# marbl/parsnp

Hardware: AMD Instinct MI355X
Metric: genomes/sec (MUM+LCB end-to-end) (higher is better)
Workload: dtype int32

## Files before the change

### parsnp_amd/csrc/engine/engine_core.h

```cpp
#pragma once
#include <algorithm>
#include <atomic>
#include <chrono>
#include <cstdint>
#include <cstdio>
#include <cstdlib>
#include <cstring>
#include <memory>
#include <mutex>
#include <new>
#include <string>
#include <thread>
#include <vector>

#include "kernels.h"
#include "store_kernels.h"
#include "dense_kernels.h"
#include "index_kernels.h"

namespace pm {

struct HostPool {
    void* (*alloc_fn)(size_t) = nullptr;
    void (*free_fn)(void*) = nullptr;
// ... 669 lines not shown
            ensure(d_okcnt, (size_t)ncand + 1); ensure(d_okpos, (size_t)ncand + 1);
            be.launch("ok_count", (int64_t)ncand + 1, OkCount{d_ok.p, ncand_p, d_okcnt.p, (int64_t)ncand});
            be.exclusive_scan(d_okcnt.p, d_okpos.p, (size_t)ncand + 1);
            const int64_t* nok_p = d_okpos.p + ncand;
            int64_t nok = 0;
            if (exact) be.d2h(&nok, nok_p, 8);
            const size_t nokz = exact ? (size_t)nok : (size_t)ncand, nqz2 = (size_t)nq, ngz = (size_t)ngen;
            ensure(d_creg, std::max<size_t>(nokz, 1)); ensure(d_ck, std::max<size_t>(nokz, 1)); ensure(d_clon, std::max<size_t>(nokz, 1));
            std::vector<int32_t> reg_h(nokz);
            out->release();
            out->kb = pool->take(4 * nokz); out->lonb = pool->take(4 * nokz);
            out->rows = want_rows; out->dirty_known = false; out->table_id = 0; out->store_base = -1;
            const int64_t ms_before = ms_count, rg_before = rg_count, lay_before = layout_rows, pkey_before = rg_pkey_init;
            bool anchor_call = false;
            if (!want_rows) {
                ensure(d_csp, std::max<size_t>(nokz * nqz2, 1)); ensure(d_cfwd, std::max<size_t>(nokz * nqz2, 1));
                be.launch("compact_sp", (int64_t)ncand * nq,
                          CompactSp{scand, d_ok.p, d_okpos.p, nq, d_ok_k.p, d_ok_lon.p, d_osp.p, d_ofwd.p, d_creg.p, d_ck.p, d_clon.p, d_csp.p, d_cfwd.p, ncand_p});
                be.mark("download");
                group_downloads();
                out->spb = pool->take(4 * nokz * nqz2); out->fwdb = pool->take(nokz * nqz2);
                be.d2h_async(out->spb.p, d_csp.p, 4 * nokz * nqz2);
                be.d2h_async(out->fwdb.p, d_cfwd.p, nokz * nqz2);
            } else {
                anchor_call = nreg == 1 && !gb && (exact ? nok >= dirty_min : anchor_guess);
                const bool keep_rows = resident && (anchor_call || from_store);
                const bool to_store = anchor_call || keep_rows;
                int32_t* p_start; uint8_t* p_strand; int32_t* p_lon; uint32_t* p_flags;
                if (to_store) {
                    if (anchor_call) { ms_count = 0; rg_count = 0; layout_rows = -1; rg_pkey_init = 0; }
                    const size_t base = (size_t)ms_count, upto = base + nokz;
                    ensure_keep(d_anchor_start, std::max<size_t>(upto * ngz, 1), base * ngz); ensure_keep(d_ms_strand, std::max<size_t>(upto * ngz, 1), base * ngz);
                    ensure_keep(d_anchor_lon, std::max<size_t>(upto, 1), base); ensure_keep(d_anchor_flags, std::max<size_t>(upto, 1), base);
                    ensure_keep(d_ms_shift, std::max<size_t>(upto, 1), base); ensure_keep(d_ms_len, std::max<size_t>(upto, 1), base); ensure_keep(d_ms_state, std::max<size_t>(upto, 1), base);
                    p_start = d_anchor_start.p + base * ngz; p_strand = d_ms_strand.p + base * ngz; p_lon = d_anchor_lon.p + base; p_flags = d_anchor_flags.p + base;
                    out->store_base = (int64_t)base;
                    ms_count = (int64_t)upto;
                } else {
                    ensure(d_csp, std::max<size_t>(nokz * ngz, 1)); ensure(d_cfwd, std::max<size_t>(nokz * ngz, 1)); ensure(d_cflags, std::max<size_t>(nokz, 1));
                    p_start = d_csp.p; p_strand = d_cfwd.p; p_lon = d_clon.p; p_flags = d_cflags.p;
                }
                const bool long_list = nreg == 1 && (exact ? nok >= dirty_min : anchor_guess);
                if (long_list) ensure(d_dirty, nokz);
                {
                    const ClearJob jobs[] = {{p_flags, 4 * nokz, 0}, {long_list ? d_dirty.p : nullptr, long_list ? 4 * nokz : 0, 0},
                                             {to_store ? d_ms_shift.p + (ms_count - (int64_t)nokz) : nullptr, to_store ? 4 * nokz : 0, 0},
                                             {to_store ? d_ms_state.p + (ms_count - (int64_t)nokz) : nullptr, to_store ? nokz : 0, 0}};
                    be.clear_many(jobs, 4);
                }
                be.launch("compact_candidates", (int64_t)ncand * ngen,
                          CompactCandidates{scand, d_ok.p, d_okpos.p, ngen, d_ok_k.p, d_ok_lon.p, d_osp.p, d_ofwd.p, d_starts.p, d_lens.p, d_glen,
                                            d_creg.p, d_ck.p, p_lon, p_start, p_strand, p_flags, ncand_p});
                if (long_list) {
                    const int64_t nblocks = ((int64_t)nokz + kDirtyBlock - 1) / kDirtyBlock, groups = (ngen + 63) / 64;
                    ensure(d_bmax, (size_t)nblocks * ngz); ensure(d_bmin, (size_t)nblocks * ngz);
                    be.launch_wave("dirty_extent", nblocks * groups, DirtyExtent{p_start, p_lon, p_flags, nok_p, ngen, d_bmax.p, d_bmin.p});
                    be.launch_wave("dirty_prefix", groups, DirtyPrefix{nblocks, ngen, d_bmax.p, d_bmin.p});
                    be.launch_wave("dirty_mark", nblocks * groups, DirtyMark{p_start, p_lon, nok_p, ngen, d_bmax.p, d_bmin.p, p_flags, d_dirty.p});
                    be.launch("dirty_merge", (int64_t)nokz, DirtyMerge{d_dirty.p, p_flags, nok_p});
                    out->dirty_known = true;
                }
                if (to_store) {
                    be.d2d(d_ms_len.p + (ms_count - (int64_t)nokz), p_lon, 4 * nokz);
                    if (anchor_call) out->table_id = ++table_counter;
                }
                be.mark("download");
                group_downloads();
                out->flagsb = pool->take(4 * nokz);
                be.d2h_async(out->flagsb.p, p_flags, 4 * nokz);
                if (!keep_rows) {
                    out->startb = pool->take(4 * nokz * ngz); out->strandb = pool->take(nokz * ngz);
                    be.d2h_async(out->startb.p, p_start, 4 * nokz * ngz);
                    be.d2h_async(out->strandb.p, p_strand, nokz * ngz);
                }
                be.d2h_async(out->lonb.p, p_lon, 4 * nokz);
            }
            if (!want_rows) be.d2h_async(out->lonb.p, d_clon.p, 4 * nokz);
            be.d2h_async(reg_h.data(), d_creg.p, 4 * nokz);
            be.d2h_async(out->kb.p, d_ck.p, 4 * nokz);
            int64_t counts_h[2] = {ncand_i, nok};
            if (!exact) { be.d2h_async(&counts_h[0], ncand_p, 8); be.d2h_async(&counts_h[1], nok_p, 8); }
            flush_downloads();
            be.mark(nullptr);
            be.sync();
            if (!exact) {
                ncand_i = counts_h[0]; nok = counts_h[1];
                const bool fits = (uint64_t)ncand_i <= ncand && anchor_call == (nreg == 1 && !gb && nok >= dirty_min);
                if (!fits) {
                    ms_count = ms_before; rg_count = rg_before; layout_rows = lay_before; rg_pkey_init = pkey_before;
                    tail_repeats++;
                    be.mark("candidates");
                    continue;
                }
                last_candidates = ncand_i;
                if (out->store_base >= 0) ms_count = out->store_base + nok;
            }
            hint.ncand = std::max<int64_t>(ncand_i, 1); hint.nok = nok;
            last_accepted = nok;
            if (anchor_call) { anchor_table_rows = nok; anchor_table_id = out->table_id; }
            for (int64_t w = 0; w < nok; w++) out->off[(size_t)reg_h[(size_t)w] + 1]++;
            for (int64_t r = 0; r < nreg; r++) out->off[(size_t)r + 1] += out->off[(size_t)r];
            out->total = out->off[(size_t)nreg];
            if (out->table_id && out->store_base == 0) anchor_flags_h.assign(out->flags(), out->flags() + nok);
            break;
        }
        collect_timing();
        return 0;
    }


    bool resident = false;
    int64_t ms_count = 0;
    int64_t rg_count = 0;
    std::vector<RegInfo> rg_info_h;
    std::vector<uint32_t> anchor_flags_h;
    static constexpr int kAgain = -6;

    void begin_store_call() { timing.clear(); last_events = last_rest = last_positions = last_candidates = last_accepted = last_grouped = last_grouped_wide = last_wide_regions = 0; last_handed_back = -1; last_index_bucketed = last_index_overflow = 0; last_index_lost = -1; last_alg[0] = last_alg[1] = last_alg[2] = 0; }
    Store store_view() { return Store{d_anchor_start.p, d_ms_strand.p, d_anchor_lon.p, d_anchor_flags.p, d_ms_shift.p, d_ms_len.p, d_ms_state.p, ngen}; }
    Layout layout_view(uint64_t* image, bool coherent = true) { return Layout{image, d_lay_off.p, d_lay_bits.p, coherent ? 1 : 0}; }
    size_t layout_geometry() {
        const size_t ngz = (size_t)ngen;
        if (lay_words == 0) {
            std::vector<int64_t> off(ngz + 1, 0), bits(ngz);
            for (size_t j = 0; j < ngz; j++) { bits[j] = glen_h[j] + 1; off[j + 1] = off[j] + (bits[j] + 63) / 64 + 1; }
            ensure(d_lay_off, ngz + 1); ensure(d_lay_bits, ngz);
            be.h2d(d_lay_off.p, off.data(), 8 * (ngz + 1)); be.h2d(d_lay_bits.p, bits.data(), 8 * ngz);
            lay_words = (size_t)off[ngz];
            lay_off_h = off;
        }
        return lay_words;
    }
    int need_resident(int64_t table_id) {
        if (!resident) { error = "the session is not in resident mode"; return -2; }
        if (table_id == 0 || table_id != anchor_table_id) { error = "the anchor table of this request is no longer resident"; return -2; }
        return 0;
    }
    int store_settle(int64_t table_id, RowInfo* out) {
        if (int rc = settle_launch(table_id)) return rc;
        return store_info(0, anchor_table_rows, out);
    }
    int settle_launch(int64_t table_id) {
        if (int rc = need_resident(table_id)) return rc;
        begin_store_call();
        const int64_t rows = anchor_table_rows;
        const size_t words = layout_geometry();
        ensure(d_image, words);
        be.mark("settle");
        ensure(d_foreign_count, 2);
        be.memset(d_foreign_count.p, 0, 16);
        ms_key_rows = 0; foreign_seen = 0;
        be.memset(d_image.p, 0, 8 * words);
        ensure(d_recwords, words);
        be.memset(d_recwords.p, 0, words);
        const Store S = store_view();
        const Layout L = layout_view(d_image.p);
        be.launch_wave("settle_clean", rows, SettleClean{S, P});
        std::vector<int32_t> fl;
        for (int64_t c = 0; c < rows; c++) { const uint32_t f = anchor_flags_h[(size_t)c]; if (!(f & (kRowBad | kRowOutside)) && (f & kRowDirty)) fl.push_back((int32_t)c); }
        const bool many_flagged = flagged_div > 1 && fl.size() * (size_t)flagged_div > (size_t)rows;
        bool ordered = true;
        for (int64_t c = 0; c < rows && ordered; c++) { const uint32_t f = anchor_flags_h[(size_t)c]; ordered = !((f & kRowEarly) && !(f & (kRowBad | kRowOutside | kRowDirty))); }
        if (ordered && !force_atomic_marks) be.launch_wave("store_mark_ordered", ((rows + kMarkRows - 1) / kMarkRows) * ((ngen + 63) / 64), StoreMarkOrdered{S, L, rows});
        else be.launch("store_mark", rows * ngen, StoreMark{S, L, 0, (uint8_t)(kStAccepted | kStFlagged), kStAccepted});
        be.launch("layout_sentinel", (int64_t)ngen, LayoutSentinel{d_lay_off.p, d_lay_bits.p, d_image.p});
        if (!fl.empty()) {
            const uint64_t* before_once = d_once.p; const uint64_t* before_twice = d_twice.p;
            ensure(d_once, words); ensure(d_twice, words); ensure(d_list, fl.size());
            if (d_once.p != before_once || d_twice.p != before_twice) { be.memset(d_once.p, 0, 8 * words); be.memset(d_twice.p, 0, 8 * words); }
            be.h2d(d_list.p, fl.data(), 4 * fl.size());
            be.launch("collide_mark", (int64_t)fl.size() * ngen, CollideMark{S, d_list.p, layout_view(d_once.p), d_twice.p});
            be.launch_wave("collide_test", (int64_t)fl.size(), CollideTest{S, d_list.p, layout_view(d_twice.p, false)});
            be.launch("collide_clear", (int64_t)fl.size() * ngen, CollideClear{S, d_list.p, layout_view(d_once.p), d_twice.p});
            ensure(d_t_rem, 2); ensure(d_t_done, fl.size());
            {
                const ClearJob jobs[] = {{d_t_rem.p, 16, 0}, {d_t_done.p, fl.size(), 0}};
                be.clear_many(jobs, 2);
            }
            be.launch("count_tangled", (int64_t)fl.size(), CountTangled{S, d_list.p, d_t_rem.p});
            if (many_flagged) {
                uint64_t tangled = 0;
                be.d2h(&tangled, d_t_rem.p, 8);
                if ((int64_t)tangled > tangled_max) {
                    be.mark(nullptr);
                    collect_timing_more();
                    error = "too many rows of the list overlap one another (rearranged genomes): the host route decides";
                    return kAgain;
                }
            }
            be.launch_wave("settle_flagged", (int64_t)fl.size(), SettleFlagged{S, layout_view(d_image.p, false), P, d_list.p});
            {
                const int32_t* before = d_owner.p;
                ensure(d_owner, words);
                if (d_owner.p != before) be.memset(d_owner.p, 0, 4 * words);
            }
            int rounds = tangle_rounds ? kTangleRounds : 0;
            if (rounds && tangle_ran > 0) {
                int last = 0;
                for (int r = 1; r < tangle_ran; r++) if (tangle_left[r] < tangle_left[r - 1]) last = r;
                rounds = std::min(kTangleRounds, last + 2);
            }
            ensure(d_t_left, kTangleRounds);
            for (int round = 0; round < rounds; round++) {
                be.launch_wave("tangle_owner", (int64_t)fl.size(), TangleOwner{S, d_list.p, d_lay_off.p, d_lay_bits.p, d_owner.p, d_t_done.p, d_t_rem.p});
                be.launch_wave("tangle_settle", (int64_t)fl.size(), TangleSettle{S, layout_view(d_image.p, false), P, d_list.p, d_owner.p, d_t_done.p, d_t_rem.p});
                be.launch_wave("tangle_clear", (int64_t)fl.size(), TangleClear{S, d_list.p, d_lay_off.p, d_lay_bits.p, d_owner.p, d_t_done.p, d_t_rem.p, d_t_left.p + round});
            }
            tangle_ran = 0;
            if (rounds) { be.d2h_async(tangle_left, d_t_left.p, 8 * (size_t)rounds); tangle_ran = rounds; }
            be.launch_wave("settle_tangled", 1, SettleTangled{S, L, P, d_list.p, (int64_t)fl.size(), d_t_done.p, d_t_rem.p});
        }
        layout_rows = rows;
        return 0;
    }
    int store_settle_seeds(int64_t table_id, int32_t q, RowInfo* out, std::vector<RegInfo>* infos, std::vector<int32_t>* ids) {
        infos->clear(); ids->clear();
// ... 500 lines not shown
            be.launch("dense_keys", n, DenseKeys{d_dstart.p, nflag, d_drank[k].p, (int64_t)1 << k, d_dkey.p, d_dval.p});
            be.sort_pairs(d_dkey.p, d_dkey2.p, d_dval.p, d_dval2.p, (size_t)n, 32 + bits_for(top_rank));
            be.launch("dense_heads", n + 1, DenseHeads{d_dkey2.p, n, d_dhead.p});
            be.exclusive_scan(d_dhead.p, d_dfirst.p, (size_t)n + 1);
            ensure(d_drank[k + 1], (size_t)n);
            be.launch("dense_rerank", n, DenseRerank{d_dval2.p, d_dhead.p, d_dfirst.p, d_drank[k + 1].p});
            L.lv[k + 1] = d_drank[k + 1].p;
            be.d2h(&groups, d_dfirst.p + n, 8);
            if (groups == n) break;
        }
        if (groups != n) { error = "suffix-array sort did not converge"; return -5; }
        dense_rounds = k + 1;
        L.top = k;
        be.launch("dense_lcp", n, DenseLcp{L, d_dval2.p, d_dstart.p, nflag, d_dlcp.p});
        be.launch("dense_rep", n, DenseRep{d_R.p, d_dlist.p, d_dval2.p, d_dstart.p, nflag, d_dlcp.p, d_rep.p});
        return 0;
    }
    bool dense_mode = false;
    std::vector<uint8_t> dense_h;
    void collect_timing_more() { for (const PhaseTime& t : be.collect()) timing.push_back(t); }

    int allgather_host(const void* send, int64_t bytes, void* recv) {
        if (!coll.device) return coll.allgather(coll.ctx, send, bytes, recv);
        ensure(d_hsend, (size_t)bytes); ensure(d_hrecv, (size_t)bytes * (size_t)coll.world);
        be.h2d(d_hsend.p, send, (size_t)bytes);
        if (be.allgather_dev(d_hsend.p, bytes, d_hrecv.p)) return 1;
        be.d2h(recv, d_hrecv.p, (size_t)bytes * (size_t)coll.world);
        return 0;
    }

    std::vector<uint64_t> ev_key_h, ev_val_h;
    std::vector<int32_t> rep_h;
    int ev_lbits = 0;
    int64_t work_budget = 1 << 22;
    int64_t dirty_min = 4096;
    int64_t flagged_div = 8;
    int64_t tangled_max = 1 << 17;
    bool fast_tail = true;
    int64_t tail_repeats = 0;
    bool tangle_rounds = true;
    bool group_small = true;
    bool group_wide = false;
    int64_t last_grouped = 0;
    int64_t last_grouped_wide = 0, last_handed_back = -1, last_wide_regions = 0;
    bool force_atomic_marks = false;
    int filter_factor = 8;
    int slot_factor = 2;
    bool bucket_sort = true;
    bool index_build = true;
    int64_t index_bucket_min = 1 << 24;
    bool index_verify = false;
    int64_t index_overflow_cap = 0;
    int64_t last_index_bucketed = 0, last_index_overflow = 0, last_index_lost = -1;
    bool master_seg = true;
    bool force_gate = false;
    int64_t chain_window = 4096;
    int64_t chain_passed[2] = {-1, -1};
    bool force_chain_tie = false;
    bool force_unsure = false;
    bool order_debug = false;
    int64_t outside_writes = 0;
    int64_t exact_cluster_tests = 0;
    int64_t deferred_regions = 0;
    bool clusters_out_of_order = false;
    int64_t hint_shrink = 1;
    bool phase_timing = true;
    bool tune(const std::string& key, int64_t value) {
        if (key == "flagged_div" && value >= 1) { flagged_div = value; return true; }
        if (key == "tangled_max" && value >= 0) { tangled_max = value; return true; }
        if (key == "tangle_rounds") { tangle_rounds = value != 0; return true; }
        if (key == "fast_tail") { fast_tail = value != 0; return true; }
        if (key == "atomic_marks") { force_atomic_marks = value != 0; return true; }
        if (key == "master_seg") { master_seg = value != 0; return true; }
        if (key == "bucket_sort") { bucket_sort = value != 0; return true; }
        if (key == "index_build") { index_build = value != 0; return true; }
        if (key == "index_bucket_min" && value >= 1) { index_bucket_min = value; return true; }
        if (key == "index_verify") { index_verify = value != 0; return true; }
        if (key == "index_overflow_cap" && value >= 0) { index_overflow_cap = value; return true; }
        if (key == "filter_factor") { filter_factor = value < 1 ? 1 : (int)value; return true; }
        if (key == "slot_factor") { slot_factor = value < 1 ? 1 : (int)value; return true; }
        if (key == "stage_gate") { force_gate = value != 0; return true; }
        if (key == "chain_window" && value >= 1 && value <= kChainWindowMax) { chain_window = value; return true; }
        if (key == "chain_tie") { force_chain_tie = value != 0; return true; }
        if (key == "cluster_unsure") { force_unsure = value != 0; return true; }
        if (key == "order_debug") { order_debug = value != 0; return true; }
        if (key == "timing") { phase_timing = value != 0; be.timing_on = phase_timing; return true; }
        if (key == "group_small") { group_small = value != 0; return true; }
        if (key == "group_wide") { group_wide = value != 0; return true; }
        if (key == "work_budget" && value > 0) { work_budget = value; return true; }
        if (key == "dense_all") { dense_all = value != 0; return true; }
        if (key == "dirty_min" && value >= 0) { dirty_min = value; return true; }
        if (key == "hint_shrink" && value >= 1) { hint_shrink = value; return true; }
        if (key == "copy_kernel") { return tune_copy_kernel(be, value != 0, 0); }
        return false;
    }

    void release() {
        if (chain_event) { be.event_wait(chain_event); be.event_release(chain_event); chain_event = nullptr; }
        for (BufBase* b : all_bufs) { if (b->raw) be.free(b->raw); b->raw = nullptr; b->cap = 0; }
        if (chain_host) be.pinned_free(chain_host);
        chain_host = nullptr; chain_host_cap = 0; chain_pending = false;
        if (blk) be.free(blk);
        if (d_goff) be.free(d_goff);
        if (d_glen) be.free(d_glen);
        blk = nullptr; d_goff = nullptr; d_glen = nullptr;
    }

    struct DeviceOutOfMemory { size_t bytes; };

private:
    B& be;
    struct BufBase { void* raw = nullptr; size_t cap = 0; };
    std::vector<BufBase*> all_bufs;
    template <class T> struct Buf : BufBase {
        T* p = nullptr;
    };
    template <class T> void ensure(Buf<T>& b, size_t n) {
        if (n <= b.cap && b.p) return;
        if (std::find(all_bufs.begin(), all_bufs.end(), (BufBase*)&b) == all_bufs.end()) all_bufs.push_back(&b);
        if (b.raw) be.free(b.raw);
        b.raw = nullptr; b.p = nullptr; b.cap = 0;
        const size_t want = n + n / 4 + 16;
        b.raw = be.alloc(want * sizeof(T));
        if (!b.raw) throw DeviceOutOfMemory{want * sizeof(T)};
        b.p = (T*)b.raw; b.cap = want;
    }
    template <class T> void ensure_keep(Buf<T>& b, size_t n, size_t keep) {
        if (n <= b.cap && b.p) return;
        if (std::find(all_bufs.begin(), all_bufs.end(), (BufBase*)&b) == all_bufs.end()) all_bufs.push_back(&b);
        const size_t want = n + n / 2 + 16;
        void* raw = be.alloc(want * sizeof(T));
        if (!raw) throw DeviceOutOfMemory{want * sizeof(T)};
        if (b.p && keep) { be.d2d(raw, b.p, keep * sizeof(T)); be.sync(); }
        if (b.raw) be.free(b.raw);
        b.raw = raw; b.p = (T*)raw; b.cap = want;
    }
    void collect_timing() { timing = be.collect(); }
    template <class T> static auto group_on(T& b, int) -> decltype(b.d2h_group(), void()) { b.d2h_group(); }
    template <class T> static void group_on(T&, long) {}
    template <class T> static auto flush_on(T& b, int) -> decltype(b.d2h_flush(), void()) { b.d2h_flush(); }
    template <class T> static void flush_on(T&, long) {}
    template <class T> static auto tune_copy_kernel(T& b, bool on, int) -> decltype(b.group_copies = on, true) { b.group_copies = on; return true; }
    template <class T> static bool tune_copy_kernel(T&, bool, long) { return true; }
    template <class T> static auto sort_keys_on(T& b, uint64_t* ki, uint64_t* ko, size_t n, int lo, int hi, int) -> decltype(b.sort_keys(ki, ko, n, lo, hi), true) { b.sort_keys(ki, ko, n, lo, hi); return true; }
    template <class T> static bool sort_keys_on(T&, uint64_t*, uint64_t*, size_t, int, int, long) { return false; }
    void group_downloads() { group_on(be, 0); }
    void flush_downloads() { flush_on(be, 0); }

    SeqBlock* blk = nullptr; int64_t* d_goff = nullptr; int64_t* d_glen = nullptr;
    int64_t total_words = 0;
    Packed P{};
    size_t ev_cap_hint = 0, cand_cap_hint = 0, rest_cap_hint[2] = {0, 0}, grp_cap_hint = 0;
    struct CallHint { int64_t units = 0, ncand = 0, nok = 0; };
    std::vector<CallHint> call_hints;
    int64_t call_ordinal = 0;
    Buf<uint8_t> d_gflag; Buf<int64_t> d_glo;
    Buf<int64_t> d_bkbase, d_bkbegin, d_ovf; Buf<uint64_t> d_ikey, d_ikey2, d_ikey3, d_ikey4;
    Buf<RegionInfo> d_R; Buf<int64_t> d_starts, d_lens, d_posbase;
    Buf<uint64_t> d_slots; Buf<uint32_t> d_filter, d_repeated; Buf<int32_t> d_next, d_rep, d_run, d_epm;
    Buf<int64_t> d_ucount, d_uoff; Buf<UnitRec> d_units;
    Buf<uint64_t> d_counter, d_evkey, d_evval, d_evkey2, d_evval2, d_evkey3, d_evval3; Buf<int64_t> d_sliceoff;
    Buf<int64_t> d_lo, d_cov; Buf<EventAtK> d_state; Buf<PairState> d_wsummary; Buf<int32_t> d_emax;
    Buf<uint64_t> d_cand; Buf<GenomeAtK> d_at; Buf<uint8_t> d_ok; Buf<int32_t> d_ok_k, d_ok_lon, d_osp; Buf<uint8_t> d_ofwd;
    Buf<uint64_t> d_wmask; Buf<int64_t> d_wcount, d_woff;
    Buf<int64_t> d_bcount, d_bbegin, d_pbase;
    Buf<int64_t> d_okcnt, d_okpos, d_cbase; Buf<int32_t> d_coarse; Buf<int32_t> d_creg, d_ck, d_clon, d_csp; Buf<uint8_t> d_cfwd;
    Buf<uint32_t> d_cflags, d_dirty; Buf<int32_t> d_bmax, d_bmin;
    Buf<GenomeAtK> d_xsend, d_xrecv; Buf<uint8_t> d_hsend, d_hrecv;
    Buf<RestItem> d_rest; Buf<uint64_t> d_qcount;
    Buf<uint8_t> d_dense; Buf<int32_t> d_dfi, d_dlist, d_dlcp; Buf<int64_t> d_dstart, d_dhead, d_dfirst;
    Buf<uint64_t> d_dkey, d_dkey2, d_dval, d_dval2; Buf<uint32_t> d_drank[kDenseMaxLevels];
    Buf<int32_t> d_anchor_start, d_anchor_lon; Buf<uint32_t> d_anchor_flags;
    int64_t table_counter = 0;
    Buf<uint64_t> d_image;
    Buf<uint8_t> d_ms_strand, d_ms_state, d_small8, d_o_strand; Buf<int32_t> d_ms_shift, d_ms_len, d_list, d_list2, d_j_min, d_j_max, d_o_start;
    Buf<int64_t> d_rg_start, d_rg_len, d_lay_off, d_lay_bits, d_v_row0, d_v_first, d_f_start, d_f_end, d_f_pack; Buf<RegInfo> d_rg_info; Buf<uint64_t> d_rg_count, d_once, d_twice;
    Buf<RowInfo> d_rowinfo; Buf<uint64_t> d_alg;
    Buf<int64_t> d_sd_cnt, d_sd_off; Buf<uint8_t> d_sd_keep;
    Buf<uint64_t> d_t_rem; Buf<uint8_t> d_t_done;
    Buf<int32_t> d_v_done, d_owner; Buf<uint8_t> d_v_defer, d_v_involved;
    Buf<uint64_t> d_t_left; uint64_t tangle_left[8] = {0, 0, 0, 0, 0, 0, 0, 0}; int tangle_ran = 0;
    Buf<int64_t> d_rg_pkey; Buf<OutsideWrite> d_outw; Buf<uint64_t> d_outw_count; int64_t rg_pkey_init = 0; uint64_t outside_writes_call = 0;
    Buf<ForeignRead> d_foreign; Buf<uint64_t> d_foreign_count, d_foreign_masks; Buf<int64_t> d_ms_key;
    size_t foreign_cap = 0; int64_t ms_key_rows = 0; uint64_t foreign_seen = 0;
    static constexpr size_t kHitCap = 256;
    Buf<uint64_t> d_hit_count, d_hit_owned, d_hit_present; Buf<int32_t> d_hits; Buf<uint8_t> d_recwords;
    Buf<int64_t> d_ch_flag, d_ch_pos, d_ch_head, d_ch_hpos, d_ch_survive, d_ch_spos, d_ch_hdr;
    Buf<uint64_t> d_ch_key, d_ch_val, d_ch_skey, d_ch_srow, d_ch_key2, d_ch_row2, d_ch_lcblen;
    Buf<uint8_t> d_ch_verdict, d_ch_outhead; Buf<int32_t> d_ch_outrow;
    Buf<int64_t> d_ch_back, d_ch_wflag, d_ch_wpos, d_ch_wlist, d_ch_wend; Buf<uint8_t> d_ch_wverdict, d_ch_wkeep;
    uint8_t* chain_host = nullptr; size_t chain_host_cap = 0; void* chain_event = nullptr; bool chain_pending = false; int64_t chain_cap = 0;
    size_t lay_words = 0, rg_cap_hint = 0;
    int64_t layout_rows = -1;
};

}
```

### parsnp_amd/csrc/engine/kernels.h

```cpp
#pragma once
#include <cstdint>

#if defined(__HIPCC__)
#define PM_HD __host__ __device__ inline
#else
#define PM_HD inline
#endif

namespace pm {

PM_HD int ctz64(uint64_t x) {
#if defined(__HIP_DEVICE_COMPILE__)
    return __ffsll((unsigned long long)x) - 1;
#else
    return __builtin_ctzll(x);
#endif
}
PM_HD int clz64(uint64_t x) {
#if defined(__HIP_DEVICE_COMPILE__)
    return __clzll((long long)x);
#else
    return __builtin_clzll(x);
#endif
}
// ... 1626 lines not shown
    PM_HD void operator()(int64_t c) const { cnt[c] = (c < *ncand && c < cap) ? (ok[c] ? 1 : 0) : 0; }
};
struct CompactSp {
    const uint64_t* cand; const uint8_t* ok; const int64_t* pos; int32_t nq;
    const int32_t* k; const int32_t* lon; const int32_t* sp; const uint8_t* fwd;
    int32_t* out_region; int32_t* out_k; int32_t* out_lon; int32_t* out_sp; uint8_t* out_fwd;
    const int64_t* ncand;
    PM_HD void operator()(int64_t tid) const {
        const int64_t c = tid / nq; const int g = (int)(tid % nq);
        if (c >= *ncand || !ok[c]) return;
        const int64_t w = pos[c];
        out_sp[w * nq + g] = sp[tid]; out_fwd[w * nq + g] = fwd[tid];
        if (g == 0) { out_region[w] = (int32_t)(cand[c] >> 32); out_k[w] = k[c]; out_lon[w] = lon[c]; }
    }
};
constexpr uint32_t kRowBad = 1;
constexpr uint32_t kRowOutside = 2;
constexpr uint32_t kRowReverse = 4;
constexpr uint32_t kRowDirty = 8;
constexpr uint32_t kRowEarly = 16;
struct CompactCandidates {
    const uint64_t* cand; const uint8_t* ok; const int64_t* pos; int32_t ngen;
    const int32_t* k; const int32_t* lon; const int32_t* sp; const uint8_t* fwd;
    const int64_t* starts; const int64_t* lens; const int64_t* glen;
    int32_t* out_region; int32_t* out_k; int32_t* out_lon; int32_t* out_start; uint8_t* out_strand; uint32_t* out_flags;
    const int64_t* ncand;
    PM_HD void operator()(int64_t tid) const {
        const int64_t c = tid / ngen; const int j = (int)(tid % ngen);
        if (c >= *ncand || !ok[c]) return;
        const int64_t w = pos[c];
        const int64_t r = (int64_t)(cand[c] >> 32);
        const int64_t lo = lon[c];
        const int64_t ws = starts[r * ngen + j], wl = lens[r * ngen + j];
        int64_t st; uint32_t f, bits = 0;
        if (j == 0) {
            st = (int64_t)k[c] + ws; f = 1;
            if ((uint64_t)k[c] + 1 > (uint64_t)(uint32_t)wl) bits |= kRowBad;
            out_region[w] = (int32_t)r; out_k[w] = k[c]; out_lon[w] = lon[c];
        } else {
            const int64_t q = sp[c * (ngen - 1) + j - 1];
            f = fwd[c * (ngen - 1) + j - 1];
            if ((uint64_t)q + 1 > (uint64_t)(uint32_t)wl) bits |= kRowBad;
            const int64_t at = q + ws;
            st = f ? at : glen[j] - (at + lo);
            if (!f) bits |= kRowReverse;
        }
        if (st + lo > glen[j] || st < 0) bits |= kRowOutside;
        out_start[w * ngen + j] = (int32_t)st; out_strand[w * ngen + j] = (uint8_t)f;
        if (bits) atomic_or32(&out_flags[w], bits);
    }
};

constexpr int kDirtyBlock = 256;
PM_HD bool row_marks(uint32_t flags, int32_t lon) { return !(flags & (kRowBad | kRowOutside)) && lon >= 5; }
struct DirtyExtent {
    const int32_t* start; const int32_t* lon; const uint32_t* flags; const int64_t* n_live; int32_t ngen; int32_t* bmax; int32_t* bmin;
    PM_HD void wave(int64_t w) const {
        const int64_t n = *n_live;
        const int64_t groups = (ngen + 63) / 64, blk = w / groups; const int g0 = (int)(w % groups) * 64;
        const int64_t c0 = blk * kDirtyBlock, c1 = c0 + kDirtyBlock < n ? c0 + kDirtyBlock : n;
#if defined(__HIP_DEVICE_COMPILE__)
        const int j = g0 + (int)__lane_id();
        if (j >= ngen) return;
        int32_t mx = -1, mn = 0x7fffffff;
#pragma unroll 8
        for (int64_t c = c0; c < c1; c++) {
            const int32_t a = start[c * ngen + j], l = lon[c];
            if (!row_marks(flags[c], l)) continue;
            if (a + l > mx) mx = a + l;
            if (a < mn) mn = a;
        }
        bmax[blk * ngen + j] = mx; bmin[blk * ngen + j] = mn;
#else
        for (int j = g0; j < g0 + 64 && j < ngen; j++) {
            int32_t mx = -1, mn = 0x7fffffff;
            for (int64_t c = c0; c < c1; c++) {
                const int32_t a = start[c * ngen + j], l = lon[c];
                if (!row_marks(flags[c], l)) continue;
                if (a + l > mx) mx = a + l;
                if (a < mn) mn = a;
            }
            bmax[blk * ngen + j] = mx; bmin[blk * ngen + j] = mn;
        }
#endif
    }
};
struct DirtyPrefix {
    int64_t nblocks; int32_t ngen; int32_t* bmax; int32_t* bmin;
    PM_HD void wave(int64_t w) const {
#if defined(__HIP_DEVICE_COMPILE__)
        const int j0 = (int)w * 64 + (int)__lane_id(), j1 = j0 + 1;
        if (j0 >= ngen) return;
#else
        const int j0 = (int)w * 64, j1 = j0 + 64 < ngen ? j0 + 64 : ngen;
#endif
        for (int j = j0; j < j1; j++) {
            int32_t mx = -1, mn = 0x7fffffff;
            for (int64_t b0 = 0; b0 < nblocks; b0 += 16) {
                int32_t x[16], y[16];
#pragma unroll
                for (int u = 0; u < 16; u++) { const int64_t b = b0 + u < nblocks ? b0 + u : nblocks - 1; x[u] = bmax[b * ngen + j]; y[u] = bmin[b * ngen + j]; }
#pragma unroll
                for (int u = 0; u < 16; u++) {
                    if (b0 + u >= nblocks) continue;
                    bmax[(b0 + u) * ngen + j] = mx; bmin[(b0 + u) * ngen + j] = mn;
                    if (x[u] > mx) mx = x[u];
                    if (y[u] < mn) mn = y[u];
                }
            }
        }
    }
};
struct DirtyMark {
    const int32_t* start; const int32_t* lon; const int64_t* n_live; int32_t ngen; const int32_t* bmax; const int32_t* bmin;
    const uint32_t* flags; uint32_t* dirty;
    PM_HD void wave(int64_t w) const {
        const int64_t n = *n_live;
        const int64_t groups = (ngen + 63) / 64, blk = w / groups; const int g0 = (int)(w % groups) * 64;
        const int64_t c0 = blk * kDirtyBlock, c1 = c0 + kDirtyBlock < n ? c0 + kDirtyBlock : n;
#if defined(__HIP_DEVICE_COMPILE__)
        const int j = g0 + (int)__lane_id();
        const bool act = j < ngen;
        const int jj = act ? j : 0;
        int32_t mx = act ? bmax[blk * ngen + j] : -1, mn = act ? bmin[blk * ngen + j] : 0x7fffffff;
        for (int64_t cb = c0; cb < c1; cb += 8) {
            int32_t a[8], l[8]; uint32_t fl[8];
#pragma unroll
            for (int u = 0; u < 8; u++) {
                const int64_t c = cb + u < c1 ? cb + u : c1 - 1;
                a[u] = start[c * ngen + jj]; l[u] = lon[c]; fl[u] = flags[c];
            }
#pragma unroll
            for (int u = 0; u < 8; u++) {
                if (cb + u >= c1 || !row_marks(fl[u], l[u])) continue;
                const int32_t b = a[u] + l[u];
                const bool early = act && !(a[u] >= mx);
                const bool hit = early && !(b <= mn);
                if (act) { if (b > mx) mx = b; if (a[u] < mn) mn = a[u]; }
                const unsigned long long any_early = __ballot(early), any_hit = __ballot(hit);
                if (any_early && __lane_id() == 0) atomic_or32(&dirty[cb + u], kRowEarly | (any_hit ? kRowDirty : 0u));
            }
        }
#else
        for (int j = g0; j < g0 + 64 && j < ngen; j++) {
            int32_t mx = bmax[blk * ngen + j], mn = bmin[blk * ngen + j];
            for (int64_t c = c0; c < c1; c++) {
                const int32_t l = lon[c];
                if (!row_marks(flags[c], l)) continue;
                const int32_t a = start[c * ngen + j], b = a + l;
                if (!(a >= mx)) dirty[c] |= kRowEarly | (!(b <= mn) ? kRowDirty : 0u);
                if (b > mx) mx = b;
                if (a < mn) mn = a;
            }
        }
#endif
    }
};
struct DirtyMerge {
    const uint32_t* dirty; uint32_t* flags; const int64_t* n_live;
    PM_HD void operator()(int64_t c) const { if (c < *n_live && dirty[c]) flags[c] |= dirty[c] & (kRowDirty | kRowEarly); }
};

}
```

### parsnp_amd/csrc/engine/store_kernels.h

```cpp
#pragma once
#include "kernels.h"

namespace pm {

#if defined(__HIP_DEVICE_COMPILE__)
template <class F> __device__ inline void lanes_for(int from, int n, F f) {
    for (int j = (from & ~63) + (int)__lane_id(); j < n; j += 64) if (j >= from) f(j);
}
__device__ inline int32_t wave_min_i32(int32_t x) { for (int d = 32; d >= 1; d >>= 1) { const int32_t y = __shfl_xor(x, d, 64); if (y < x) x = y; } return x; }
__device__ inline int32_t wave_max_i32(int32_t x) { for (int d = 32; d >= 1; d >>= 1) { const int32_t y = __shfl_xor(x, d, 64); if (y > x) x = y; } return x; }
__device__ inline uint32_t wave_or_u32(uint32_t x) { for (int d = 32; d >= 1; d >>= 1) x |= (uint32_t)__shfl_xor((int)x, d, 64); return x; }
__device__ inline int32_t wave_bcast_i32(int32_t x, int lane) { return __shfl(x, lane, 64); }
__device__ inline uint64_t wave_or_u64(uint64_t x) { return ((uint64_t)wave_or_u32((uint32_t)(x >> 32)) << 32) | wave_or_u32((uint32_t)x); }
__device__ inline uint64_t wave_sum_u64(uint64_t x) {
    for (int d = 32; d >= 1; d >>= 1) x += ((uint64_t)(uint32_t)__shfl_xor((int)(x >> 32), d, 64) << 32) | (uint32_t)__shfl_xor((int)(uint32_t)x, d, 64);
    return x;
}
__device__ inline bool wave_leader() { return __lane_id() == 0; }
__device__ inline void wave_sync() { __syncthreads(); }
#define PM_WAVE_SHARED __shared__
__device__ inline uint64_t load_coherent64(const uint64_t* p) { return __hip_atomic_load(p, __ATOMIC_RELAXED, __HIP_MEMORY_SCOPE_AGENT); }
__device__ inline int32_t load_coherent32(const int32_t* p) { return __hip_atomic_load(p, __ATOMIC_RELAXED, __HIP_MEMORY_SCOPE_AGENT); }
__device__ inline uint8_t load_coherent8(const uint8_t* p) { return __hip_atomic_load(p, __ATOMIC_RELAXED, __HIP_MEMORY_SCOPE_AGENT); }
__device__ inline void store_coherent32(int32_t* p, int32_t v) { __hip_atomic_store(p, v, __ATOMIC_RELAXED, __HIP_MEMORY_SCOPE_AGENT); }
// ... 215 lines not shown
        lanes_for(from, n, [&](int j) {
            if (j >= first) return;
            const int64_t s = (int64_t)st[j] + dl;
            const int32_t l = img_run_up(L, j, s, len);
            const int32_t r = l < len ? img_run_down(L, j, s + len - 1, len - l) : 0;
            if ((l | r) != 0) { first = j; tl = l; tr = r; }
        });
        const int32_t F = wave_min_i32(first);
        if (F == 0x7fffffff) break;
        tl = wave_bcast_i32(tl, F & 63); tr = wave_bcast_i32(tr, F & 63);
        dl += tl; len -= tl + tr; from = F + 1;
    }
    *pdl = dl; *plen = len;
    if (len < 2 || n <= 1) return false;
    if (!S.strand[c * n]) return false;
    if (f & kRowReverse) {
        uint32_t bad = 0;
        const int64_t r0 = P.goff[0] + (int64_t)st[0] + dl;
        lanes_for(0, n, [&](int j) {
            if (S.strand[c * n + j]) return;
            const int64_t l1 = (int64_t)st[j] + dl;
            if (lce_fwd(P, P.goff[2 * j + 1] + (P.glen[j] - l1 - len), r0, len) != len) bad = 1;
        });
        if (wave_or_u32(bad)) return false;
    }
    return true;
}

struct SettleClean {
    Store S; Packed P;
    PM_HD void wave(int64_t c) const {
        const uint32_t f = S.flags[c];
        uint8_t st = 0;
        if (!(f & kRowBad)) st = (uint8_t)(kStBuilt | ((f & kRowOutside) ? 0 : kStOk) | ((f & kRowDirty) ? kStFlagged : 0));
        int32_t dl = 0, len = S.lon[c];
        if ((st & (kStBuilt | kStOk | kStFlagged)) == (kStBuilt | kStOk)) {
            Layout none{nullptr, nullptr, nullptr, 0};
            if (settle_row(S, none, P, c, false, &dl, &len)) st |= kStAccepted;
            dl = 0; len = S.lon[c];
        }
        if (wave_leader()) { S.state[c] = st; S.shift[c] = 0; S.len[c] = len; }
    }
};
struct StoreMark {
    Store S; Layout L; int64_t row0; uint8_t mask, want;
    PM_HD void operator()(int64_t tid) const {
        const int64_t c = row0 + tid / S.ngen; const int j = (int)(tid % S.ngen);
        if ((S.state[c] & mask) != want) return;
        const int64_t a = (int64_t)S.start[c * S.ngen + j] + S.shift[c];
        img_set_range(L, j, a, a + S.len[c]);
    }
};
constexpr int kMarkRows = 256;
struct StoreMarkOrdered {
    Store S; Layout L; int64_t rows;
    PM_HD void wave(int64_t w) const {
        const int n = S.ngen;
        const int64_t groups = (n + 63) / 64, blk = w / groups;
        const int g0 = (int)(w % groups) * 64;
        const int64_t c0 = blk * kMarkRows, c1 = c0 + kMarkRows < rows ? c0 + kMarkRows : rows;
        lanes_for(g0, g0 + 64 < n ? g0 + 64 : n, [&](int j) {
            uint64_t* img = L.image + L.word_off[j];
            const int64_t nb = L.nbits[j];
            int64_t cur = -1; uint64_t bits = 0; bool first = true;
            auto flush = [&](bool last) {
                if (cur < 0) return;
                if (first || last) atomic_or64(&img[cur], bits); else img[cur] = bits;
                first = false;
            };
            for (int64_t cb = c0; cb < c1; cb += 8) {
                int32_t a[8], l[8]; uint8_t st[8];
#pragma unroll
                for (int u = 0; u < 8; u++) {
                    const int64_t c = cb + u < c1 ? cb + u : c1 - 1;
                    a[u] = S.start[c * n + j]; l[u] = S.len[c]; st[u] = S.state[c];
                }
#pragma unroll
                for (int u = 0; u < 8; u++) {
                    if (cb + u >= c1 || (st[u] & (kStAccepted | kStFlagged)) != kStAccepted) continue;
                    int64_t x = a[u], e = x + l[u];
                    if (x < 0) x = 0;
                    if (e > nb) e = nb;
                    while (x < e) {
                        const int64_t wi = x >> 6;
                        if (wi != cur) { flush(false); cur = wi; bits = 0; }
                        const int lo = (int)(x & 63);
                        const int64_t span = (64 - lo) < (e - x) ? (64 - lo) : (e - x);
                        bits |= (span == 64 ? ~0ull : ((1ull << span) - 1)) << lo;
                        x += span;
                    }
                }
            }
            flush(true);
        });
    }
};
struct StoreUnmark {
    Store S; Layout L; const int32_t* rows;
    PM_HD void operator()(int64_t tid) const {
        const int64_t c = rows[tid / S.ngen]; const int j = (int)(tid % S.ngen);
        const int64_t a = (int64_t)S.start[c * S.ngen + j] + S.shift[c];
        img_clear_range(L, j, a, a + S.len[c]);
    }
};

struct CollideMark {
    Store S; const int32_t* list; Layout once; uint64_t* twice;
    PM_HD void operator()(int64_t tid) const {
        const int64_t c = list[tid / S.ngen]; const int j = (int)(tid % S.ngen);
        int64_t a = S.start[c * S.ngen + j], b = a + S.lon[c];
        if (a < 0) a = 0;
        if (b > once.nbits[j]) b = once.nbits[j];
        const int64_t base = once.word_off[j];
        while (a < b) {
            const int lo = (int)(a & 63);
            const int64_t span = (64 - lo) < (b - a) ? (64 - lo) : (b - a);
            const uint64_t mask = (span == 64 ? ~0ull : ((1ull << span) - 1)) << lo;
            const uint64_t old = atomic_fetch_or64(&once.image[base + (a >> 6)], mask);
            if (old & mask) atomic_or64(&twice[base + (a >> 6)], old & mask);
            a += span;
        }
    }
};
struct CollideTest {
    Store S; const int32_t* list; Layout twice;
    PM_HD void wave(int64_t i) const {
        const int64_t c = list[i];
        const int n = S.ngen;
        uint32_t hit = 0;
        lanes_for(0, n, [&](int j) {
            const int64_t a = S.start[c * n + j];
            if (img_any(twice, j, a, a + S.lon[c])) hit = 1;
        });
        if (wave_or_u32(hit) && wave_leader()) S.state[c] |= kStTangled;
    }
};
struct CountTangled {
    Store S; const int32_t* list; uint64_t* count;
    PM_HD void operator()(int64_t i) const { if (S.state[list[i]] & kStTangled) atomic_add64(count, 1); }
};
struct CollideClear {
    Store S; const int32_t* list; Layout once; uint64_t* twice;
    PM_HD void operator()(int64_t tid) const {
        const int64_t c = list[tid / S.ngen]; const int j = (int)(tid % S.ngen);
        int64_t a = S.start[c * S.ngen + j], b = a + S.lon[c];
        if (a < 0) a = 0;
        if (b > once.nbits[j]) b = once.nbits[j];
        const int64_t base = once.word_off[j];
        for (int64_t w = a >> 6; a < b && w <= ((b - 1) >> 6); w++) { once.image[base + w] = 0; twice[base + w] = 0; }
// ... 1486 lines not shown
```

Before: 31160.

## Shorten per-wave row walks in dirty-extent and ordered store-mark kernels

Adds a default-on row_walks mode that shrinks the rows each wave walks: dirty-extent blocks drop from 256 to 32 rows and ordered store marking from 256 to 128 rows. To keep the serial prefix short, it becomes two-level, with per-chunk prefixes over 64 blocks plus a carry pass whose result DirtyMark merges in. The short store-mark variant also software-prefetches the next 8 start values. The aim is more waves in flight and shorter serial latency chains, at the cost of extra launches, more boundary atomics and extra scratch buffers.

```diff
diff --git a/parsnp_amd/csrc/engine/engine_core.h b/parsnp_amd/csrc/engine/engine_core.h
--- a/parsnp_amd/csrc/engine/engine_core.h
+++ b/parsnp_amd/csrc/engine/engine_core.h
@@ -745,11 +745,21 @@
                           CompactCandidates{scand, d_ok.p, d_okpos.p, ngen, d_ok_k.p, d_ok_lon.p, d_osp.p, d_ofwd.p, d_starts.p, d_lens.p, d_glen,
                                             d_creg.p, d_ck.p, p_lon, p_start, p_strand, p_flags, ncand_p});
                 if (long_list) {
-                    const int64_t nblocks = ((int64_t)nokz + kDirtyBlock - 1) / kDirtyBlock, groups = (ngen + 63) / 64;
+                    const int64_t block = row_walks ? kWalkBlock : kDirtyBlock;
+                    const int64_t nblocks = ((int64_t)nokz + block - 1) / block, groups = (ngen + 63) / 64;
                     ensure(d_bmax, (size_t)nblocks * ngz); ensure(d_bmin, (size_t)nblocks * ngz);
-                    be.launch_wave("dirty_extent", nblocks * groups, DirtyExtent{p_start, p_lon, p_flags, nok_p, ngen, d_bmax.p, d_bmin.p});
-                    be.launch_wave("dirty_prefix", groups, DirtyPrefix{nblocks, ngen, d_bmax.p, d_bmin.p});
-                    be.launch_wave("dirty_mark", nblocks * groups, DirtyMark{p_start, p_lon, nok_p, ngen, d_bmax.p, d_bmin.p, p_flags, d_dirty.p});
+                    if (row_walks) {
+                        const int64_t nchunks = (nblocks + kWalkChunk - 1) / kWalkChunk;
+                        ensure(d_cmax, (size_t)nchunks * ngz); ensure(d_cmin, (size_t)nchunks * ngz);
+                        be.launch_wave("dirty_extent_short", nblocks * groups, DirtyExtentShort{{p_start, p_lon, p_flags, nok_p, ngen, d_bmax.p, d_bmin.p}});
+                        be.launch_wave("dirty_chunk", nchunks * groups, DirtyChunk{nblocks, ngen, d_bmax.p, d_bmin.p, d_cmax.p, d_cmin.p});
+                        be.launch_wave("dirty_carry", groups, DirtyPrefix{nchunks, ngen, d_cmax.p, d_cmin.p});
+                        be.launch_wave("dirty_mark_short", nblocks * groups, DirtyMarkShort{{p_start, p_lon, nok_p, ngen, d_bmax.p, d_bmin.p, p_flags, d_dirty.p, d_cmax.p, d_cmin.p}});
+                    } else {
+                        be.launch_wave("dirty_extent", nblocks * groups, DirtyExtent{{p_start, p_lon, p_flags, nok_p, ngen, d_bmax.p, d_bmin.p}});
+                        be.launch_wave("dirty_prefix", groups, DirtyPrefix{nblocks, ngen, d_bmax.p, d_bmin.p});
+                        be.launch_wave("dirty_mark", nblocks * groups, DirtyMark{{p_start, p_lon, nok_p, ngen, d_bmax.p, d_bmin.p, p_flags, d_dirty.p}});
+                    }
                     be.launch("dirty_merge", (int64_t)nokz, DirtyMerge{d_dirty.p, p_flags, nok_p});
                     out->dirty_known = true;
                 }
@@ -854,7 +864,8 @@
         const bool many_flagged = flagged_div > 1 && fl.size() * (size_t)flagged_div > (size_t)rows;
         bool ordered = true;
         for (int64_t c = 0; c < rows && ordered; c++) { const uint32_t f = anchor_flags_h[(size_t)c]; ordered = !((f & kRowEarly) && !(f & (kRowBad | kRowOutside | kRowDirty))); }
-        if (ordered && !force_atomic_marks) be.launch_wave("store_mark_ordered", ((rows + kMarkRows - 1) / kMarkRows) * ((ngen + 63) / 64), StoreMarkOrdered{S, L, rows});
+        if (ordered && !force_atomic_marks && row_walks) be.launch_wave("store_mark_ordered", ((rows + kWalkRows - 1) / kWalkRows) * ((ngen + 63) / 64), StoreMarkOrderedShort{{S, L, rows}});
+        else if (ordered && !force_atomic_marks) be.launch_wave("store_mark_ordered", ((rows + kMarkRows - 1) / kMarkRows) * ((ngen + 63) / 64), StoreMarkOrdered{{S, L, rows}});
         else be.launch("store_mark", rows * ngen, StoreMark{S, L, 0, (uint8_t)(kStAccepted | kStFlagged), kStAccepted});
         be.launch("layout_sentinel", (int64_t)ngen, LayoutSentinel{d_lay_off.p, d_lay_bits.p, d_image.p});
         if (!fl.empty()) {
@@ -1461,6 +1472,7 @@
     bool index_verify = false;
     int64_t index_overflow_cap = 0;
     int64_t last_index_bucketed = 0, last_index_overflow = 0, last_index_lost = -1;
+    bool row_walks = true;
     bool master_seg = true;
     bool force_gate = false;
     int64_t chain_window = 4096;
@@ -1483,6 +1495,7 @@
         if (key == "master_seg") { master_seg = value != 0; return true; }
         if (key == "bucket_sort") { bucket_sort = value != 0; return true; }
         if (key == "index_build") { index_build = value != 0; return true; }
+        if (key == "row_walks") { row_walks = value != 0; return true; }
         if (key == "index_bucket_min" && value >= 1) { index_bucket_min = value; return true; }
         if (key == "index_verify") { index_verify = value != 0; return true; }
         if (key == "index_overflow_cap" && value >= 0) { index_overflow_cap = value; return true; }
@@ -1574,7 +1587,7 @@
     Buf<uint64_t> d_wmask; Buf<int64_t> d_wcount, d_woff;
     Buf<int64_t> d_bcount, d_bbegin, d_pbase;
     Buf<int64_t> d_okcnt, d_okpos, d_cbase; Buf<int32_t> d_coarse; Buf<int32_t> d_creg, d_ck, d_clon, d_csp; Buf<uint8_t> d_cfwd;
-    Buf<uint32_t> d_cflags, d_dirty; Buf<int32_t> d_bmax, d_bmin;
+    Buf<uint32_t> d_cflags, d_dirty; Buf<int32_t> d_bmax, d_bmin, d_cmax, d_cmin;
     Buf<GenomeAtK> d_xsend, d_xrecv; Buf<uint8_t> d_hsend, d_hrecv;
     Buf<RestItem> d_rest; Buf<uint64_t> d_qcount;
     Buf<uint8_t> d_dense; Buf<int32_t> d_dfi, d_dlist, d_dlcp; Buf<int64_t> d_dstart, d_dhead, d_dfirst;
diff --git a/parsnp_amd/csrc/engine/kernels.h b/parsnp_amd/csrc/engine/kernels.h
--- a/parsnp_amd/csrc/engine/kernels.h
+++ b/parsnp_amd/csrc/engine/kernels.h
@@ -1702,13 +1702,18 @@
 };
 
 constexpr int kDirtyBlock = 256;
+#ifndef PM_WALK_BLOCK
+#define PM_WALK_BLOCK 32
+#endif
+constexpr int kWalkBlock = PM_WALK_BLOCK;
+constexpr int kWalkChunk = 64;
 PM_HD bool row_marks(uint32_t flags, int32_t lon) { return !(flags & (kRowBad | kRowOutside)) && lon >= 5; }
-struct DirtyExtent {
+template <int B> struct DirtyExtentOf {
     const int32_t* start; const int32_t* lon; const uint32_t* flags; const int64_t* n_live; int32_t ngen; int32_t* bmax; int32_t* bmin;
     PM_HD void wave(int64_t w) const {
         const int64_t n = *n_live;
         const int64_t groups = (ngen + 63) / 64, blk = w / groups; const int g0 = (int)(w % groups) * 64;
-        const int64_t c0 = blk * kDirtyBlock, c1 = c0 + kDirtyBlock < n ? c0 + kDirtyBlock : n;
+        const int64_t c0 = blk * B, c1 = c0 + B < n ? c0 + B : n;
 #if defined(__HIP_DEVICE_COMPILE__)
         const int j = g0 + (int)__lane_id();
         if (j >= ngen) return;
@@ -1735,6 +1740,24 @@
 #endif
     }
 };
+struct DirtyExtent : DirtyExtentOf<kDirtyBlock> {};
+struct DirtyExtentShort : DirtyExtentOf<kWalkBlock> {};
+PM_HD void extent_prefix(int32_t* bmax, int32_t* bmin, int32_t ngen, int j, int64_t b0, int64_t b1, int32_t* pmx, int32_t* pmn) {
+    int32_t mx = -1, mn = 0x7fffffff;
+    for (int64_t r0 = b0; r0 < b1; r0 += 16) {
+        int32_t x[16], y[16];
+#pragma unroll
+        for (int u = 0; u < 16; u++) { const int64_t b = r0 + u < b1 ? r0 + u : b1 - 1; x[u] = bmax[b * ngen + j]; y[u] = bmin[b * ngen + j]; }
+#pragma unroll
+        for (int u = 0; u < 16; u++) {
+            if (r0 + u >= b1) continue;
+            bmax[(r0 + u) * ngen + j] = mx; bmin[(r0 + u) * ngen + j] = mn;
+            if (x[u] > mx) mx = x[u];
+            if (y[u] < mn) mn = y[u];
+        }
+    }
+    *pmx = mx; *pmn = mn;
+}
 struct DirtyPrefix {
     int64_t nblocks; int32_t ngen; int32_t* bmax; int32_t* bmin;
     PM_HD void wave(int64_t w) const {
@@ -1744,35 +1767,48 @@
 #else
         const int j0 = (int)w * 64, j1 = j0 + 64 < ngen ? j0 + 64 : ngen;
 #endif
+        for (int j = j0; j < j1; j++) { int32_t mx, mn; extent_prefix(bmax, bmin, ngen, j, 0, nblocks, &mx, &mn); }
+    }
+};
+struct DirtyChunk {
+    int64_t nblocks; int32_t ngen; int32_t* bmax; int32_t* bmin; int32_t* cmax; int32_t* cmin;
+    PM_HD void wave(int64_t w) const {
+        const int64_t groups = (ngen + 63) / 64, chunk = w / groups;
+        const int64_t b0 = chunk * kWalkChunk, b1 = b0 + kWalkChunk < nblocks ? b0 + kWalkChunk : nblocks;
+#if defined(__HIP_DEVICE_COMPILE__)
+        const int j0 = (int)(w % groups) * 64 + (int)__lane_id(), j1 = j0 + 1;
+        if (j0 >= ngen) return;
+#else
+        const int j0 = (int)(w % groups) * 64, j1 = j0 + 64 < ngen ? j0 + 64 : ngen;
+#endif
         for (int j = j0; j < j1; j++) {
-            int32_t mx = -1, mn = 0x7fffffff;
-            for (int64_t b0 = 0; b0 < nblocks; b0 += 16) {
-                int32_t x[16], y[16];
-#pragma unroll
-                for (int u = 0; u < 16; u++) { const int64_t b = b0 + u < nblocks ? b0 + u : nblocks - 1; x[u] = bmax[b * ngen + j]; y[u] = bmin[b * ngen + j]; }
-#pragma unroll
-                for (int u = 0; u < 16; u++) {
-                    if (b0 + u >= nblocks) continue;
-                    bmax[(b0 + u) * ngen + j] = mx; bmin[(b0 + u) * ngen + j] = mn;
-                    if (x[u] > mx) mx = x[u];
-                    if (y[u] < mn) mn = y[u];
-                }
-            }
-        }
-    }
-};
-struct DirtyMark {
+            int32_t mx, mn;
+            extent_prefix(bmax, bmin, ngen, j, b0, b1, &mx, &mn);
+            cmax[chunk * ngen + j] = mx; cmin[chunk * ngen + j] = mn;
+        }
+    }
+};
+template <int B> struct DirtyMarkOf {
     const int32_t* start; const int32_t* lon; const int64_t* n_live; int32_t ngen; const int32_t* bmax; const int32_t* bmin;
     const uint32_t* flags; uint32_t* dirty;
+    const int32_t* cmax; const int32_t* cmin;
+    PM_HD void carry_in(int64_t blk, int j, int32_t* mx, int32_t* mn) const {
+        *mx = bmax[blk * ngen + j]; *mn = bmin[blk * ngen + j];
+        if (!cmax) return;
+        const int32_t x = cmax[blk / kWalkChunk * ngen + j], y = cmin[blk / kWalkChunk * ngen + j];
+        if (x > *mx) *mx = x;
+        if (y < *mn) *mn = y;
+    }
     PM_HD void wave(int64_t w) const {
         const int64_t n = *n_live;
         const int64_t groups = (ngen + 63) / 64, blk = w / groups; const int g0 = (int)(w % groups) * 64;
-        const int64_t c0 = blk * kDirtyBlock, c1 = c0 + kDirtyBlock < n ? c0 + kDirtyBlock : n;
+        const int64_t c0 = blk * B, c1 = c0 + B < n ? c0 + B : n;
 #if defined(__HIP_DEVICE_COMPILE__)
         const int j = g0 + (int)__lane_id();
         const bool act = j < ngen;
         const int jj = act ? j : 0;
-        int32_t mx = act ? bmax[blk * ngen + j] : -1, mn = act ? bmin[blk * ngen + j] : 0x7fffffff;
+        int32_t mx = -1, mn = 0x7fffffff;
+        if (act) carry_in(blk, j, &mx, &mn);
         for (int64_t cb = c0; cb < c1; cb += 8) {
             int32_t a[8], l[8]; uint32_t fl[8];
 #pragma unroll
@@ -1793,7 +1829,8 @@
         }
 #else
         for (int j = g0; j < g0 + 64 && j < ngen; j++) {
-            int32_t mx = bmax[blk * ngen + j], mn = bmin[blk * ngen + j];
+            int32_t mx, mn;
+            carry_in(blk, j, &mx, &mn);
             for (int64_t c = c0; c < c1; c++) {
                 const int32_t l = lon[c];
                 if (!row_marks(flags[c], l)) continue;
@@ -1806,6 +1843,8 @@
 #endif
     }
 };
+struct DirtyMark : DirtyMarkOf<kDirtyBlock> {};
+struct DirtyMarkShort : DirtyMarkOf<kWalkBlock> {};
 struct DirtyMerge {
     const uint32_t* dirty; uint32_t* flags; const int64_t* n_live;
     PM_HD void operator()(int64_t c) const { if (c < *n_live && dirty[c]) flags[c] |= dirty[c] & (kRowDirty | kRowEarly); }
diff --git a/parsnp_amd/csrc/engine/store_kernels.h b/parsnp_amd/csrc/engine/store_kernels.h
--- a/parsnp_amd/csrc/engine/store_kernels.h
+++ b/parsnp_amd/csrc/engine/store_kernels.h
@@ -291,13 +291,17 @@
     }
 };
 constexpr int kMarkRows = 256;
-struct StoreMarkOrdered {
+#ifndef PM_WALK_ROWS
+#define PM_WALK_ROWS 128
+#endif
+constexpr int kWalkRows = PM_WALK_ROWS;
+template <int W, bool Ahead> struct StoreMarkOrderedOf {
     Store S; Layout L; int64_t rows;
     PM_HD void wave(int64_t w) const {
         const int n = S.ngen;
         const int64_t groups = (n + 63) / 64, blk = w / groups;
         const int g0 = (int)(w % groups) * 64;
-        const int64_t c0 = blk * kMarkRows, c1 = c0 + kMarkRows < rows ? c0 + kMarkRows : rows;
+        const int64_t c0 = blk * W, c1 = c0 + W < rows ? c0 + W : rows;
         lanes_for(g0, g0 + 64 < n ? g0 + 64 : n, [&](int j) {
             uint64_t* img = L.image + L.word_off[j];
             const int64_t nb = L.nbits[j];
@@ -307,12 +311,21 @@
                 if (first || last) atomic_or64(&img[cur], bits); else img[cur] = bits;
                 first = false;
             };
+            int32_t na[8];
+            if (Ahead) {
+#pragma unroll
+                for (int u = 0; u < 8; u++) na[u] = S.start[(c0 + u < c1 ? c0 + u : c1 - 1) * n + j];
+            }
             for (int64_t cb = c0; cb < c1; cb += 8) {
                 int32_t a[8], l[8]; uint8_t st[8];
 #pragma unroll
                 for (int u = 0; u < 8; u++) {
                     const int64_t c = cb + u < c1 ? cb + u : c1 - 1;
-                    a[u] = S.start[c * n + j]; l[u] = S.len[c]; st[u] = S.state[c];
+                    a[u] = Ahead ? na[u] : S.start[c * n + j]; l[u] = S.len[c]; st[u] = S.state[c];
+                }
+                if (Ahead && cb + 8 < c1) {
+#pragma unroll
+                    for (int u = 0; u < 8; u++) na[u] = S.start[(cb + 8 + u < c1 ? cb + 8 + u : c1 - 1) * n + j];
                 }
 #pragma unroll
                 for (int u = 0; u < 8; u++) {
@@ -334,6 +347,8 @@
         });
     }
 };
+struct StoreMarkOrdered : StoreMarkOrderedOf<kMarkRows, false> {};
+struct StoreMarkOrderedShort : StoreMarkOrderedOf<kWalkRows, true> {};
 struct StoreUnmark {
     Store S; Layout L; const int32_t* rows;
     PM_HD void operator()(int64_t tid) const {
```

New measurement: 31720 (median of 6 runs). +1.8%, better.
